# evenrose/CMDIAD

Measured on AMD Instinct MI355X. Metric: images/sec end-to-end (extract+distill+kNN score), higher is better.
Workload: dtype bf16; 1 GPU; configs[1]: DINO ViT-B/8 + Point-MAE predict (DoubleRGBPointFeatures: both modalities are extracted, this method has no distillation step at test time; the `mtfi_step` leg times the method that has one), 224x224 RGB + 24576-point clouds (1024 groups x 128), batch 32/GPU, bagel-sized banks (xyz 76518x768, rgb 19129x768); batch_per_gpu=32, rotating_input_batches=4, bank=single, hip_graphs=True, search_operands=bf16 (fp32 accumulate, exact fp32 re-score of the winner), weights=seeded random init (no checkpoints offline)

## Files before the change

cmdiad_amd/csrc/blocks.cpp:

```cpp
#include "common.h"

extern "C" size_t cmdiad_transformer_block_workspace_bytes(int M, int C, int hidden)
{
    if (M <= 0 || C <= 0 || hidden <= 0) return 0;
    const size_t rows256 = ((size_t)M + 255) / 256 * 256;
    return (size_t)M * (size_t)(2 * C + hidden) * sizeof(uint16_t)
         + (size_t)(C / 64) * M * 2 * sizeof(float)
         + rows256 * sizeof(float);
}

extern "C" int cmdiad_transformer_block_fwd(float* x, const float* pos, const cmdiad_block_weights* w, int B, int T, int C, int H,
                                            int hidden, float eps, int flags, uint16_t* q, uint16_t* k, uint16_t* vt, void* workspace,
                                            size_t workspace_bytes, cmdiad_stream_t stream)
{
    CMDIAD_REQUIRE(x && w && q && k && vt && workspace, CMDIAD_ERR_ARG, "cmdiad_transformer_block_fwd: null pointer");
    CMDIAD_REQUIRE(B > 0 && T > 0 && C > 0 && H > 0 && C == H * 64 && hidden > 0, CMDIAD_ERR_ARG,
                   "cmdiad_transformer_block_fwd: need C == 64*H (B=%d T=%d C=%d H=%d hidden=%d)", B, T, C, H, hidden);
    const int M = B * T;
    CMDIAD_REQUIRE(workspace_bytes >= cmdiad_transformer_block_workspace_bytes(M, C, hidden), CMDIAD_ERR_WORKSPACE,
                   "cmdiad_transformer_block_fwd: workspace %zu < %zu bytes", workspace_bytes,
                   cmdiad_transformer_block_workspace_bytes(M, C, hidden));
    const bool folded = w->qkv_wf != nullptr;
    CMDIAD_REQUIRE(folded ? (w->qkv_bf && w->fc1_wf && w->fc1_bf) : (!w->qkv_bf && !w->fc1_wf && !w->fc1_bf), CMDIAD_ERR_ARG,
                   "cmdiad_transformer_block_fwd: the folded weights come as all four or none");
    CMDIAD_REQUIRE((flags & ~(CMDIAD_BLOCK_LN1_READY | CMDIAD_BLOCK_PREP_NEXT)) == 0 && (folded || flags == 0), CMDIAD_ERR_ARG,
                   "cmdiad_transformer_block_fwd: flags %d need the folded weights", flags);
    uint16_t* h = (uint16_t*)workspace;
    uint16_t* a = h + (size_t)M * C;
    uint16_t* m = a + (size_t)M * C;
    float* part = (float*)(m + (size_t)M * hidden);
    float* rstd = part + (size_t)(C / 64) * M * 2;
    int rc;
    if (flags & CMDIAD_BLOCK_LN1_READY) {
        if ((rc = cmdiad_gemm_qkv(h, w->qkv_wf, w->qkv_bf, rstd, B, T, C, q, k, vt, stream))) return rc;
    } else {
        if ((rc = cmdiad_layernorm(x, pos, w->ln1_w, w->ln1_b, eps, M, C, h, nullptr, 0, nullptr, nullptr, stream))) return rc;
        if ((rc = cmdiad_gemm_qkv(h, w->qkv_w, w->qkv_b, nullptr, B, T, C, q, k, vt, stream))) return rc;
    }
    if ((rc = cmdiad_attention(q, k, vt, B, H, T, a, stream))) return rc;
    cmdiad_gemm_args g{};
    g.A = a; g.lda = C; g.W = w->proj_w; g.ldw = C; g.M = M; g.N = C; g.K = C; g.bias = w->proj_b;
    g.residual = x; g.ldr = C; g.out_f32 = x; g.ldo32 = C; g.act = CMDIAD_ACT_NONE; g.group_rows = 1; g.split_k = 1;
    if (folded) { g.ln_xb = h; g.ld_xb = C; g.ln_part = part; }
    if ((rc = cmdiad_gemm_bf16(&g, stream))) return rc;
    cmdiad_gemm_args f1{};
    f1.A = h; f1.lda = C; f1.ldw = C; f1.M = M; f1.N = hidden; f1.K = C;
    f1.act = CMDIAD_ACT_GELU; f1.out_bf16 = m; f1.ldo16 = hidden; f1.group_rows = 1; f1.split_k = 1;
    if (folded) {
        if ((rc = cmdiad_ln_stats_finalize(part, M, C / 64, eps, rstd, nullptr, stream))) return rc;
        f1.W = w->fc1_wf; f1.bias = w->fc1_bf; f1.row_scale = rstd;
    } else {
        if ((rc = cmdiad_layernorm(x, nullptr, w->ln2_w, w->ln2_b, eps, M, C, h, nullptr, 0, nullptr, nullptr, stream))) return rc;
        f1.W = w->fc1_w; f1.bias = w->fc1_b;
    }
    if ((rc = cmdiad_gemm_bf16(&f1, stream))) return rc;
    cmdiad_gemm_args f2{};
    f2.A = m; f2.lda = hidden; f2.W = w->fc2_w; f2.ldw = hidden; f2.M = M; f2.N = C; f2.K = hidden; f2.bias = w->fc2_b;
    f2.residual = x; f2.ldr = C; f2.out_f32 = x; f2.ldo32 = C; f2.act = CMDIAD_ACT_NONE; f2.group_rows = 1; f2.split_k = 1;
    if (flags & CMDIAD_BLOCK_PREP_NEXT) { f2.ln_xb = h; f2.ld_xb = C; f2.ln_part = part; f2.add2 = pos; f2.ld_add2 = C; }
    if ((rc = cmdiad_gemm_bf16(&f2, stream))) return rc;
    if (flags & CMDIAD_BLOCK_PREP_NEXT) return cmdiad_ln_stats_finalize(part, M, C / 64, eps, rstd, nullptr, stream);
    return CMDIAD_OK;
}
```

Measured before the change: 1485 images/s.

## Fuse Point-MAE MLP fc1+GELU+fc2 into one kernel keeping hidden in LDS

For Point-MAE blocks (C=384, hidden=1536, large M) the fc1+GELU and fc2 GEMMs are replaced by a single kernel. Each workgroup owns 128 rows, streams weight pieces through a 6-slot LDS ring, computes 64-wide hidden chunks into LDS and accumulates fc2 in registers. The epilogue writes the residual and the next block's LN inputs and partial stats. This removes the bf16 hidden activation round trip through HBM and one launch, at the cost of one workgroup per CU (160KB LDS) and hand-tuned waitcnt scheduling.

Result: faster. 1509 images/s (median of 6 runs) (+1.6%).

```diff
diff --git a/cmdiad_amd/csrc/blocks.cpp b/cmdiad_amd/csrc/blocks.cpp
--- a/cmdiad_amd/csrc/blocks.cpp
+++ b/cmdiad_amd/csrc/blocks.cpp
@@ -1,4 +1,17 @@
+#include <stdlib.h>
+
 #include "common.h"
+
+int cmdiad_pmae_mlp_fused(float* x, const uint16_t* xb, const float* rstd, const uint16_t* w1, const float* b1, const uint16_t* w2,
+                          const float* b2, int M, uint16_t* ln_xb, float* ln_part, const float* add2, cmdiad_stream_t stream);
+
+static bool pmae_mlp_fused_wanted(bool folded, int M, int C, int hidden)
+{
+    if (!folded || C != 384 || hidden != 1536) return false;
+    const char* e = getenv("CMDIAD_PMAE_MLP");
+    if (e) return e[0] != '0';
+    return M >= 192 * 128;
+}
 
 extern "C" size_t cmdiad_transformer_block_workspace_bytes(int M, int C, int hidden)
 {
@@ -43,6 +56,14 @@
     g.residual = x; g.ldr = C; g.out_f32 = x; g.ldo32 = C; g.act = CMDIAD_ACT_NONE; g.group_rows = 1; g.split_k = 1;
     if (folded) { g.ln_xb = h; g.ld_xb = C; g.ln_part = part; }
     if ((rc = cmdiad_gemm_bf16(&g, stream))) return rc;
+    if (pmae_mlp_fused_wanted(folded, M, C, hidden)) {
+        if ((rc = cmdiad_ln_stats_finalize(part, M, C / 64, eps, rstd, nullptr, stream))) return rc;
+        const bool prep = flags & CMDIAD_BLOCK_PREP_NEXT;
+        if ((rc = cmdiad_pmae_mlp_fused(x, h, rstd, w->fc1_wf, w->fc1_bf, w->fc2_w, w->fc2_b, M, prep ? h : nullptr, prep ? part : nullptr,
+                                        prep ? pos : nullptr, stream))) return rc;
+        if (prep) return cmdiad_ln_stats_finalize(part, M, C / 64, eps, rstd, nullptr, stream);
+        return CMDIAD_OK;
+    }
     cmdiad_gemm_args f1{};
     f1.A = h; f1.lda = C; f1.ldw = C; f1.M = M; f1.N = hidden; f1.K = C;
     f1.act = CMDIAD_ACT_GELU; f1.out_bf16 = m; f1.ldo16 = hidden; f1.group_rows = 1; f1.split_k = 1;
diff --git a/cmdiad_amd/csrc/mlp_fused.hip b/cmdiad_amd/csrc/mlp_fused.hip
--- /dev/null
+++ b/cmdiad_amd/csrc/mlp_fused.hip
@@ -0,0 +1,245 @@
+#include <stdlib.h>
+
+#include <mutex>
+
+#include "gemm_core.h"
+
+namespace {
+
+using namespace gemm;
+
+constexpr int kC = 384, kHid = 1536, kBM = 128, kWaves = 8;
+constexpr int kChunks = kHid / 64;
+constexpr int kKT1 = kC / BK;
+constexpr int kPer = kKT1 + kC / 64;
+constexpr int kSlots = 6, kAhead = kSlots - 1;
+static_assert(kPer % kSlots == 0, "the slot of a piece depends on its place in the chunk only");
+constexpr int kPieceBytes = 64 * BK * 2;
+constexpr int kXbWave = kKT1 * 16 * BK * 2;
+constexpr int kHOff = kWaves * kXbWave;
+constexpr int kRingOff = kHOff + kWaves * 2048;
+constexpr int kLdsBytes = kRingOff + kSlots * kPieceBytes;
+static_assert(kLdsBytes == 160 * 1024, "LDS budget");
+
+struct MlpParams {
+    int M;
+    const bf16_t* xb;
+    const float* row_scale;
+    const bf16_t* w1;
+    const float* b1;
+    const bf16_t* w2;
+    const float* b2;
+    float* x;
+    bf16_t* ln_xb;
+    float* ln_part;
+    const float* add2;
+};
+
+__device__ __forceinline__ void mlp_barrier() { asm volatile("s_barrier" ::: "memory"); }
+
+__device__ __forceinline__ float half_row_sum8(float v)
+{
+    v += __builtin_bit_cast(float, __builtin_amdgcn_update_dpp(0, __builtin_bit_cast(int, v), 0xB1, 0xF, 0xF, false));
+    v += __builtin_bit_cast(float, __builtin_amdgcn_update_dpp(0, __builtin_bit_cast(int, v), 0x4E, 0xF, 0xF, false));
+    v += __builtin_bit_cast(float, __builtin_amdgcn_update_dpp(0, __builtin_bit_cast(int, v), 0x141, 0xF, 0xF, false));
+    return v;
+}
+
+template <bool LN_OUT>
+__global__ __launch_bounds__(512, 1) void pmae_mlp_fused_kernel(MlpParams p)
+{
+    extern __shared__ __attribute__((aligned(16))) char lds[];
+    const int lane = threadIdx.x & 63, wave = __builtin_amdgcn_readfirstlane(threadIdx.x >> 6);
+    const int g = lane >> 4, r16 = lane & 15;
+    const int mw = (int)blockIdx.x * kBM + wave * 16;
+    char* xs = lds + wave * kXbWave;
+    char* hs = lds + kHOff + wave * 2048;
+    char* ring = lds + kRingOff;
+
+    float rsc;
+    f32x4 b1v[4];
+    auto load_b1 = [&](int c) {
+        const float* bp = p.b1 + c * 64 + g * 4;
+#pragma unroll
+        for (int j = 0; j < 4; ++j) asm volatile("global_load_dwordx4 %0, %1, off" : "=v"(b1v[j]) : "v"(bp + j * 16) : "memory");
+    };
+    {
+        const float* rp = p.row_scale + min(mw + r16, p.M - 1);
+        asm volatile("global_load_dword %0, %1, off" : "=v"(rsc) : "v"(rp) : "memory");
+    }
+    load_b1(0);
+    const int sw_chunk = (lane & 7) ^ (lane >> 3);
+#pragma unroll
+    for (int e = 0; e < 2; ++e) {
+        const bf16_t* src = p.xb + (size_t)min(mw + e * 8 + (lane >> 3), p.M - 1) * kC + sw_chunk * 8;
+#pragma unroll
+        for (int s = 0; s < kKT1; ++s)
+            __builtin_amdgcn_global_load_lds((const __attribute__((address_space(1))) void*)(src + s * BK),
+                                             (__attribute__((address_space(3))) void*)(xs + s * 2048 + e * 1024), 16, 0, 0);
+    }
+    const char* w1l = reinterpret_cast<const char*>(p.w1 + (size_t)(wave * 8 + (lane >> 3)) * kC + sw_chunk * 8);
+    const char* w2l = reinterpret_cast<const char*>(p.w2 + (size_t)(wave * 8 + (lane >> 3)) * kHid + sw_chunk * 8);
+    auto issue = [&](int c, int q) {
+        const char* src = q < kKT1 ? w1l + ((size_t)c * 64 * kC + q * BK) * 2 : w2l + ((size_t)(q - kKT1) * 64 * kHid + c * BK) * 2;
+        __builtin_amdgcn_global_load_lds((const __attribute__((address_space(1))) void*)src,
+                                         (__attribute__((address_space(3))) void*)(ring + (q % kSlots) * kPieceBytes + wave * 1024), 16, 0, 0);
+    };
+#pragma unroll
+    for (int q = 0; q < kAhead; ++q) issue(0, q);
+    asm volatile("s_waitcnt vmcnt(4)" ::: "memory");
+    mlp_barrier();
+
+    auto ldf = [&](const char* tile, int row, int kk) { return *reinterpret_cast<const bf16x8*>(tile + lds_off(row, kk * 4 + g)); };
+    auto step = [&](const char* wt, const bf16x8& a0, const bf16x8& a1, f32x4 (&acc)[4]) {
+        bf16x8 wf[2][4];
+#pragma unroll
+        for (int kk = 0; kk < 2; ++kk)
+#pragma unroll
+            for (int j = 0; j < 4; ++j) wf[kk][j] = ldf(wt, j * 16 + r16, kk);
+        __builtin_amdgcn_s_setprio(1);
+#pragma unroll
+        for (int kk = 0; kk < 2; ++kk)
+#pragma unroll
+            for (int j = 0; j < 4; ++j) acc[j] = mfma16(wf[kk][j], kk ? a1 : a0, acc[j]);
+        __builtin_amdgcn_s_setprio(0);
+    };
+
+    f32x4 acc2[kC / 64][4];
+#pragma unroll
+    for (int nb = 0; nb < kC / 64; ++nb)
+#pragma unroll
+        for (int j = 0; j < 4; ++j) acc2[nb][j] = f32x4{0.f, 0.f, 0.f, 0.f};
+
+    for (int c = 0; c < kChunks; ++c) {
+        f32x4 acc1[4];
+#pragma unroll
+        for (int j = 0; j < 4; ++j) acc1[j] = f32x4{0.f, 0.f, 0.f, 0.f};
+        bf16x8 h0, h1;
+#pragma unroll
+        for (int q = 0; q < kPer; ++q) {
+            const int qn = q + kAhead < kPer ? q + kAhead : q + kAhead - kPer;
+            const int cn = q + kAhead < kPer ? c : c + 1;
+            const bool more = cn < kChunks;
+            if (q == 7 && more) load_b1(c + 1);
+            if (more) issue(cn, qn);
+            const char* wt = ring + (q % kSlots) * kPieceBytes;
+            if (q < kKT1) step(wt, ldf(xs + q * 2048, r16, 0), ldf(xs + q * 2048, r16, 1), acc1);
+            else step(wt, h0, h1, acc2[q - kKT1]);
+            if (!more) asm volatile("s_waitcnt vmcnt(0)" ::: "memory");
+            else if (q >= 7 && q <= 10) asm volatile("s_waitcnt vmcnt(8)" ::: "memory");
+            else asm volatile("s_waitcnt vmcnt(4)" ::: "memory");
+            mlp_barrier();
+            if (q == kKT1 - 1) {
+                __builtin_amdgcn_sched_barrier(0);
+#pragma unroll
+                for (int j = 0; j < 4; ++j) {
+                    f32x4 v = __builtin_elementwise_fma(acc1[j], f32x4{rsc, rsc, rsc, rsc}, b1v[j]);
+                    v = gelu_erf4(v);
+                    const bf16x4 hv = {f2bf(v[0]), f2bf(v[1]), f2bf(v[2]), f2bf(v[3])};
+                    *reinterpret_cast<bf16x4*>(hs + lds_off(r16, 2 * j + (g >> 1)) + (g & 1) * 8) = hv;
+                }
+                h0 = ldf(hs, r16, 0);
+                h1 = ldf(hs, r16, 1);
+            }
+        }
+    }
+
+    RowStore32 rs;
+    rs.init(hs, lane);
+    const bool full = mw + 16 <= p.M;
+    const int m0r = mw + rs.R;
+    const int ma = min(m0r, p.M - 1), mb = min(m0r + 8, p.M - 1);
+#pragma unroll
+    for (int nb = 0; nb < kC / 64; ++nb) {
+        const int n0 = nb * 64;
+        f32x4 bj[4];
+#pragma unroll
+        for (int j = 0; j < 4; ++j) bj[j] = *reinterpret_cast<const f32x4*>(p.b2 + n0 + j * 16 + g * 4);
+        f32x4 o0[2], o1[2];
+#pragma unroll
+        for (int ch = 0; ch < 2; ++ch) {
+            const int col = n0 + ch * 32 + rs.u * 4;
+            const f32x4 r0 = *reinterpret_cast<const f32x4*>(p.x + (size_t)ma * kC + col);
+            const f32x4 r1 = *reinterpret_cast<const f32x4*>(p.x + (size_t)mb * kC + col);
+            f32x4 a0 = {0.f, 0.f, 0.f, 0.f}, a1 = a0;
+            if (LN_OUT && p.add2) {
+                a0 = *reinterpret_cast<const f32x4*>(p.add2 + (size_t)ma * kC + col);
+                a1 = *reinterpret_cast<const f32x4*>(p.add2 + (size_t)mb * kC + col);
+            }
+            rs.park(acc2[nb][2 * ch] + bj[2 * ch], acc2[nb][2 * ch + 1] + bj[2 * ch + 1]);
+            f32x4 t0, t1;
+            rs.fetch(t0, t1);
+            o0[ch] = t0 + r0;
+            o1[ch] = t1 + r1;
+            if (LN_OUT && p.add2) { o0[ch] += a0; o1[ch] += a1; }
+            if (full || m0r < p.M) *reinterpret_cast<f32x4*>(p.x + (size_t)m0r * kC + col) = o0[ch];
+            if (full || m0r + 8 < p.M) *reinterpret_cast<f32x4*>(p.x + (size_t)(m0r + 8) * kC + col) = o1[ch];
+            if constexpr (LN_OUT) {
+                const bf16x4 v0 = {f2bf(o0[ch][0]), f2bf(o0[ch][1]), f2bf(o0[ch][2]), f2bf(o0[ch][3])};
+                const bf16x4 v1 = {f2bf(o1[ch][0]), f2bf(o1[ch][1]), f2bf(o1[ch][2]), f2bf(o1[ch][3])};
+                if (full || m0r < p.M) *reinterpret_cast<bf16x4*>(p.ln_xb + (size_t)m0r * kC + col) = v0;
+                if (full || m0r + 8 < p.M) *reinterpret_cast<bf16x4*>(p.ln_xb + (size_t)(m0r + 8) * kC + col) = v1;
+            }
+        }
+        if constexpr (LN_OUT) {
+            float s0 = 0.f, s1 = 0.f;
+#pragma unroll
+            for (int ch = 0; ch < 2; ++ch)
+#pragma unroll
+                for (int q = 0; q < 4; ++q) { s0 += o0[ch][q]; s1 += o1[ch][q]; }
+            s0 = half_row_sum8(s0);
+            s1 = half_row_sum8(s1);
+            const float c0 = s0 * (1.0f / 64), c1 = s1 * (1.0f / 64);
+            float q0 = 0.f, q1 = 0.f;
+#pragma unroll
+            for (int ch = 0; ch < 2; ++ch)
+#pragma unroll
+                for (int q = 0; q < 4; ++q) {
+                    const float d0 = o0[ch][q] - c0, d1 = o1[ch][q] - c1;
+                    q0 = fmaf(d0, d0, q0);
+                    q1 = fmaf(d1, d1, q1);
+                }
+            q0 = half_row_sum8(q0);
+            q1 = half_row_sum8(q1);
+            if (rs.u == 0) {
+                float2* part = reinterpret_cast<float2*>(p.ln_part) + (size_t)nb * p.M;
+                if (full || m0r < p.M) part[m0r] = make_float2(s0, q0);
+                if (full || m0r + 8 < p.M) part[m0r + 8] = make_float2(s1, q1);
+            }
+        }
+    }
+}
+
+}
+
+int cmdiad_pmae_mlp_fused(float* x, const uint16_t* xb, const float* rstd, const uint16_t* w1, const float* b1, const uint16_t* w2,
+                          const float* b2, int M, uint16_t* ln_xb, float* ln_part, const float* add2, cmdiad_stream_t stream)
+{
+    auto a16 = [](const void* q) { return ((uintptr_t)q & 15) == 0; };
+    CMDIAD_REQUIRE(x && xb && rstd && w1 && b1 && w2 && b2 && M > 0, CMDIAD_ERR_ARG, "cmdiad_pmae_mlp_fused: null operand");
+    CMDIAD_REQUIRE(a16(x) && a16(xb) && a16(w1) && a16(w2) && a16(b1) && a16(b2) && (!add2 || a16(add2)), CMDIAD_ERR_ARG,
+                   "cmdiad_pmae_mlp_fused: operands must be 16-byte aligned");
+    CMDIAD_REQUIRE(!ln_xb == !ln_part && (ln_xb || !add2) && (!ln_xb || (((uintptr_t)ln_xb & 7) == 0 && ((uintptr_t)ln_part & 7) == 0)),
+                   CMDIAD_ERR_ARG, "cmdiad_pmae_mlp_fused: ln_xb and ln_part come together (8-byte aligned); add2 only with them");
+    MlpParams p{M, (const bf16_t*)xb, rstd, (const bf16_t*)w1, b1, (const bf16_t*)w2, b2, x, (bf16_t*)ln_xb, ln_part, add2};
+    static std::mutex mu;
+    static bool attr[2] = {false, false};
+    auto go = [&](auto kernel, int which) -> int {
+        {
+            std::lock_guard<std::mutex> lock(mu);
+            if (!attr[which]) {
+                if (hipFuncSetAttribute((const void*)kernel, hipFuncAttributeMaxDynamicSharedMemorySize, kLdsBytes) != hipSuccess) {
+                    cmdiad_set_error("hipFuncSetAttribute(MaxDynamicSharedMemorySize=%d) failed", kLdsBytes);
+                    return CMDIAD_ERR_LAUNCH;
+                }
+                attr[which] = true;
+            }
+        }
+        hipLaunchKernelGGL(kernel, dim3((unsigned)((M + kBM - 1) / kBM)), dim3(kWaves * 64), kLdsBytes, (hipStream_t)stream, p);
+        return CMDIAD_OK;
+    };
+    const int rc = ln_xb ? go(pmae_mlp_fused_kernel<true>, 1) : go(pmae_mlp_fused_kernel<false>, 0);
+    if (rc) return rc;
+    CMDIAD_CHECK_LAUNCH();
+    return CMDIAD_OK;
+}
```
